# RmSchaffert/ACCV-Lab

Measured on AMD Instinct MI355X. Metric: heatmap frames/sec (1920x1080 fp32, ragged N_obj in [1,128], fused clear+draw), higher is better.
Workload: dtype f32

## Files before the change

accv-lab_amd/csrc/draw_heatmap.hip:

```cpp
#include <hip/hip_runtime.h>
#include <hip/hip_ext.h>

#include <algorithm>
#include <atomic>
#include <climits>
#include <cstdint>
#include <cstring>
#include <type_traits>

#include "accv_common.h"
#include "splat_common.h"
#include "splat_stamps.h"
#include "splat_tile.h"
#include "splat_small.h"
#include "splat_lanes.h"
#include "heatmap_prep.h"

namespace {

void note_dispatch(const char* kernel, int px, int r, bool clear, int sm, const dim3& grid, const dim3& block)
{
    snprintf(accv::dispatch_buffer(), 256, "%s<PX=%d,R=%d,CLEAR=%d,SM=%d> grid(%u,%u,%u) block(%u)", kernel, px, r, clear ? 1 : 0,
             sm, grid.x, grid.y, grid.z, block.x);
}

struct LaunchEvents {
    hipEvent_t start = nullptr, stop = nullptr;
};
LaunchEvents& launch_events()
{
    static thread_local LaunchEvents ev;
    return ev;
}
LaunchEvents take_launch_events()
{
    const LaunchEvents ev = launch_events();
    launch_events() = LaunchEvents{};
    return ev;
}
template <class K>
inline void launch_maybe_timed(K kernel, const dim3& grid, const dim3& block, hipStream_t stream, const LaunchEvents& ev,
                               const SplatParams& p)
{
    if (ev.start || ev.stop)
        hipExtLaunchKernelGGL(kernel, grid, block, 0, stream, ev.start, ev.stop, 0, p);
    else
        hipLaunchKernelGGL(kernel, grid, block, 0, stream, p);
}
template <class F>
void with_variant(bool clear, bool write_through, F&& f)
{
    using Plain = std::integral_constant<int, kStorePlain>;
    using WriteThrough = std::integral_constant<int, kStoreWriteThrough>;
    if (clear && write_through)
        f(std::true_type{}, WriteThrough{});
    else if (clear)
        f(std::true_type{}, Plain{});
    else if (write_through)
        f(std::false_type{}, WriteThrough{});
    else
        f(std::false_type{}, Plain{});
}

int launch_splat_small(SplatParams p, long long planes, bool clear, bool write_through, hipStream_t stream, const LaunchEvents& ev)
{
    p.tiles_x = (p.W + 127) / 128;
    p.tiles_y = (p.H + 15) / 16;
    p.n_tiles = planes * p.tiles_x * p.tiles_y;
    if (p.n_tiles == 0) return ACCV_OK;
    dim3 grid;
    p.grid3d = (planes <= 65535 && p.tiles_y <= 65535) ? 1 : 0;
    if (p.grid3d) {
        grid = dim3((unsigned)p.tiles_x, (unsigned)p.tiles_y, (unsigned)planes);
    } else {
        if (p.n_tiles > INT_MAX) return accv::fail(ACCV_EINVAL, "draw_heatmap: %lld tiles exceed the grid limit", p.n_tiles);
        grid = dim3((unsigned)p.n_tiles);
    }
    with_variant(clear, write_through, [&](auto CL, auto SM) {
        launch_maybe_timed(splat_small_kernel<CL, SM>, grid, dim3(64), stream, ev, p);
    });
    note_dispatch("splat_small_kernel", 4, 8, clear, write_through ? kStoreWriteThrough : kStorePlain, grid, dim3(64));
    return accv::check_launch("draw_heatmap small-splat kernel");
}

template <int PX, int R>
int launch_splat(SplatParams p, long long planes, bool clear, int sm, hipStream_t stream, const LaunchEvents& ev)
{
    p.tiles_x = (p.W + 32 * PX - 1) / (32 * PX);
    p.tiles_y = (p.H + 2 * R - 1) / (2 * R);
    p.n_tiles = planes * p.tiles_x * p.tiles_y;
    if (p.n_tiles == 0) return ACCV_OK;
    const int groups_x = (p.tiles_x + kWavesPerGroup - 1) / kWavesPerGroup;
    dim3 grid, block(kWavesPerGroup * 64);
    p.grid3d = (planes <= 65535 && p.tiles_y <= 65535) ? 1 : 0;
    if (p.grid3d) {
        grid = dim3((unsigned)groups_x, (unsigned)p.tiles_y, (unsigned)planes);
    } else {
        const long long groups = (p.n_tiles + kWavesPerGroup - 1) / kWavesPerGroup;
        if (groups > INT_MAX) return accv::fail(ACCV_EINVAL, "draw_heatmap: %lld tiles exceed the grid limit", p.n_tiles);
        grid = dim3((unsigned)groups);
    }
    attach_splat_stamps(p);
    if (PX == 1 || (sm == kStoreAdaptive && clear)) sm = kStorePlain;
    if (sm == kStoreAdaptive) {
        if constexpr (PX == 4) launch_maybe_timed(splat_kernel<PX, R, false, kStoreAdaptive>, grid, block, stream, ev, p);
    } else {
        with_variant(clear, sm == kStoreWriteThrough, [&](auto CL, auto SM) {
            if constexpr (PX == 4 || SM == kStorePlain) launch_maybe_timed(splat_kernel<PX, R, CL, SM>, grid, block, stream, ev, p);
        });
    }
    note_dispatch("splat_kernel", PX, R, clear, sm, grid, block);
    return accv::check_launch("draw_heatmap splat kernel");
}

long long compute_units()
{
    static std::atomic<int> cached[64];
    int dev = 0;
    if (hipGetDevice(&dev) != hipSuccess || dev < 0 || dev >= 64) return 0;
    int v = cached[dev].load(std::memory_order_relaxed);
    if (v == 0) {
        int n = 0;
        if (hipDeviceGetAttribute(&n, hipDeviceAttributeMultiprocessorCount, dev) != hipSuccess || n <= 0) return 0;
        cached[dev].store(n, std::memory_order_relaxed);
        v = n;
    }
    return v;
}

int dispatch_splat(SplatParams p, long long planes, bool clear, unsigned flags, hipStream_t stream, const LaunchEvents& ev)
{
    const bool small_hint = (flags & ACCV_HM_SMALL_RADII) != 0;
    const bool vec4 = (p.W % 4 == 0) && ((reinterpret_cast<uintptr_t>(p.hm) & 15u) == 0);
    const bool plane_fits_rsrc = (size_t)p.H * p.W * sizeof(float) < ((size_t)1 << 31);
    int nt;
    if (flags & ACCV_HM_WRITE_THROUGH)
        nt = kStoreWriteThrough;
    else if (flags & ACCV_HM_PLAIN_STORES)
        nt = kStorePlain;
    else
        nt = clear ? kStorePlain : kStoreAdaptive;
    if (nt != kStorePlain && !plane_fits_rsrc) nt = kStorePlain;
    p.dense_area = 0.75f * (float)p.H * (float)p.W;
    int rows = (flags & ACCV_HM_TILE_ROWS_16) ? 16 : 8;
    if (!(flags & (ACCV_HM_TILE_ROWS_8 | ACCV_HM_TILE_ROWS_16)) && clear && vec4 && !small_hint) {
        const long long cus = compute_units();
        const long long tx = (p.W + 127) / 128;
        const long long tiles8 = planes * tx * ((p.H + 15) / 16), tiles16 = planes * tx * ((p.H + 31) / 32);
        if (cus > 0 && tiles8 > 24 * cus && tiles16 <= 16 * cus) rows = 16;
    }
    if (!p.labels) p.labels = p.radii;
    if (!vec4) return launch_splat<1, 8>(p, planes, clear, kStorePlain, stream, ev);
    if (small_hint) return launch_splat_small(p, planes, clear, nt == kStoreWriteThrough, stream, ev);
    if (rows == 16) return launch_splat<4, 16>(p, planes, clear, nt, stream, ev);
    return launch_splat<4, 8>(p, planes, clear, nt, stream, ev);
}

int check_common(int h, int w, const char* who)
{
    if (h < 0 || w < 0) return accv::fail(ACCV_EINVAL, "%s: negative heatmap extent %dx%d", who, h, w);
    if (h > (1 << 29) || w > (1 << 29))
        return accv::fail(ACCV_EINVAL, "%s: heatmap extent %dx%d exceeds 2^29 per dimension", who, h, w);
    return ACCV_OK;
}

inline void coarse_scales_first(MultiParams& mp)
{
    std::stable_sort(mp.scale, mp.scale + mp.n_scales,
                     [](const SplatParams& a, const SplatParams& b) { return a.n_tiles < b.n_tiles; });
    long long tiles = 0;
    for (int i = 0; i < mp.n_scales; ++i) {
        mp.tile_begin[i] = tiles;
        tiles += mp.scale[i].n_tiles;
    }
    mp.tile_begin[mp.n_scales] = tiles;
}
inline void seal_tile_prefix(MultiParams& mp)
{
    for (int i = mp.n_scales + 1; i <= kMaxScales; ++i) mp.tile_begin[i] = mp.tile_begin[mp.n_scales];
}

inline int multiscale_store_mode(unsigned flags) { return (flags & ACCV_HM_WRITE_THROUGH) ? kStoreWriteThrough : kStorePlain; }

constexpr const char* kPerScaleNote = " (use the per-scale calls otherwise)";
long long setup_scales(MultiParams& mp, const SplatParams& proto, float* const* heatmaps, const int* heights, const int* widths,
                       const float* strides, int num_scales, int batch, int tile_h, unsigned flags, const char* who,
                       const char* map_note)
{
    long long tiles = 0;
    int used = 0;
    for (int i = 0; i < num_scales; ++i) {
        if (int rc = check_common(heights[i], widths[i], who)) return rc;
        if (!(strides[i] > 0.0f)) return accv::fail(ACCV_EINVAL, "%s: stride %d is not positive", who, i);
        if (heights[i] == 0 || widths[i] == 0) continue;
        if (!heatmaps[i]) return accv::fail(ACCV_EINVAL, "%s: heatmap %d is null", who, i);
        if (widths[i] % 4 != 0 || (reinterpret_cast<uintptr_t>(heatmaps[i]) & 15u) ||
            (size_t)heights[i] * widths[i] * sizeof(float) >= ((size_t)1 << 31))
            return accv::fail(ACCV_EINVAL, "%s: map %d needs a width that is a multiple of 4, a 16-byte aligned base and planes "
                                           "below 2 GiB%s", who, i, map_note);
        SplatParams& p = mp.scale[used];
        p = proto;
        p.hm = heatmaps[i];
        p.H = heights[i];
        p.W = widths[i];
        p.stride = strides[i];
        p.tiles_x = (p.W + 127) / 128;
        p.tiles_y = (p.H + tile_h - 1) / tile_h;
        p.n_tiles = (long long)batch * p.tiles_x * p.tiles_y;
        p.grid3d = 0;
        mp.tile_begin[used] = tiles;
        tiles += p.n_tiles;
        ++used;
    }
    mp.n_scales = used;
    mp.tile_begin[used] = tiles;
    if (!(flags & ACCV_HM_CALLER_SCALE_ORDER)) coarse_scales_first(mp);
    seal_tile_prefix(mp);
    return tiles;
}

int check_scale_arrays(const char* who, float* const* heatmaps, const int* heights, const int* widths, const float* strides,
                       int num_scales)
{
    if (num_scales < 1 || num_scales > kMaxScales)
        return accv::fail(ACCV_EINVAL, "%s: 1..%d scales supported, got %d", who, kMaxScales, num_scales);
    if (!heatmaps || !heights || !widths || !strides) return accv::fail(ACCV_EINVAL, "%s: null array", who);
    return ACCV_OK;
}
int check_scale_counts(const char* who, int batch, int per_sample, const char* what)
{
    if (batch < 0 || per_sample < 0) return accv::fail(ACCV_EINVAL, "%s: negative count", who);
    if (per_sample > (1 << 30)) return accv::fail(ACCV_EINVAL, "%s: more than 2^30 %s per sample", who, what);
    return ACCV_OK;
}
SplatParams multiscale_proto(const void* counts, int n_max, float diameter_to_sigma_factor, float k_scale, unsigned flags)
{
    SplatParams proto{};
    proto.counts = counts;
    proto.n_max = n_max;
    proto.factor = diameter_to_sigma_factor;
    proto.k = k_scale;
    proto.counts_i64 = (flags & ACCV_HM_COUNTS_I64) ? 1 : 0;
    return proto;
}

}

extern "C" {

int accv_draw_heatmap_time_next_launch(void* start_event, void* stop_event)
{
    launch_events() = LaunchEvents{static_cast<hipEvent_t>(start_event), static_cast<hipEvent_t>(stop_event)};
    return ACCV_OK;
}

size_t accv_draw_heatmap_flat_workspace_bytes(int num_planes, int num_objects)
{
    if (num_planes < 0 || num_objects < 0) return 0;
    return accv::align_up((size_t)num_planes * 4, 16) + accv::align_up(((size_t)num_planes + 1) * 4, 16) +
           accv::align_up((size_t)num_objects * 8, 16) + accv::align_up((size_t)num_objects * 4, 16) + 16;
}

int accv_draw_heatmap_flat_f32(float* heatmaps, int num_planes, int height, int width, const int32_t* centers,
                               const int32_t* radii, const int32_t* heatmap_idxes, int num_objects,
                               float diameter_to_sigma_factor, float k_scale, unsigned flags, void* workspace,
                               size_t workspace_bytes, void* stream_)
{
    hipStream_t stream = static_cast<hipStream_t>(stream_);
    const LaunchEvents ev = take_launch_events();
    if (int rc = check_common(height, width, "draw_heatmap")) return rc;
    if (num_planes < 0 || num_objects < 0) return accv::fail(ACCV_EINVAL, "draw_heatmap: negative count");
    if (num_objects > (1 << 30)) return accv::fail(ACCV_EINVAL, "draw_heatmap: more than 2^30 objects");
    const bool clear = (flags & ACCV_HM_CLEAR) != 0;
    if (num_planes == 0 || height == 0 || width == 0) return ACCV_OK;
    if (!heatmaps) return accv::fail(ACCV_EINVAL, "draw_heatmap: heatmap pointer is null");
    if (num_objects > 0 && (!centers || !radii || !heatmap_idxes))
        return accv::fail(ACCV_EINVAL, "draw_heatmap: null object array");
    if (num_objects == 0 && !clear) return ACCV_OK;
    const size_t need = accv_draw_heatmap_flat_workspace_bytes(num_planes, num_objects);
    if (!workspace || workspace_bytes < need || (reinterpret_cast<uintptr_t>(workspace) & 15u))
        return accv::fail(ACCV_EWORKSPACE, "draw_heatmap: workspace needs %zu aligned bytes, got %zu", need,
                          workspace_bytes);

    char* ws = static_cast<char*>(workspace);
    int* cnt = reinterpret_cast<int*>(ws);
    int* off = reinterpret_cast<int*>(ws + accv::align_up((size_t)num_planes * 4, 16));
    char* sc_raw = reinterpret_cast<char*>(off) + accv::align_up(((size_t)num_planes + 1) * 4, 16);
    int2* sorted_centers = reinterpret_cast<int2*>(sc_raw);
    int32_t* sorted_radii = reinterpret_cast<int32_t*>(sc_raw + accv::align_up((size_t)num_objects * 8, 16));

    if (num_planes <= kBinSmallPlanes && num_objects <= kBinSmallObjects) {
        hipLaunchKernelGGL(bin_small_kernel, dim3(1), dim3(1024), 0, stream, heatmap_idxes, num_objects, num_planes,
                           reinterpret_cast<const int2*>(centers), radii, off, sorted_centers, sorted_radii);
    } else {
        if (hipMemsetAsync(cnt, 0, (size_t)num_planes * 4, stream) != hipSuccess)
            return accv::fail(ACCV_ELAUNCH, "draw_heatmap: memset of the bin counters failed");
        const int nb = num_objects > 0 ? min((num_objects + 255) / 256, 1024) : 1;
        if (num_objects > 0)
            hipLaunchKernelGGL(bin_count_kernel, dim3(nb), dim3(256), 0, stream, heatmap_idxes, num_objects, num_planes, cnt);
        hipLaunchKernelGGL(bin_scan_kernel, dim3(1), dim3(1024), 0, stream, cnt, off, num_planes);
        if (num_objects > 0)
            hipLaunchKernelGGL(bin_fill_kernel, dim3(nb), dim3(256), 0, stream, heatmap_idxes, num_objects, num_planes, off,
                               cnt, reinterpret_cast<const int2*>(centers), radii, sorted_centers, sorted_radii);
    }
    if (int rc = accv::check_launch("draw_heatmap binning")) return rc;

    SplatParams p{};
    p.hm = heatmaps;
    p.centers = reinterpret_cast<const int32_t*>(sorted_centers);
    p.radii = sorted_radii;
    p.plane_off = off;
    p.H = height;
    p.W = width;
    p.factor = diameter_to_sigma_factor;
    p.k = k_scale;
    return dispatch_splat(p, num_planes, clear, flags, stream, ev);
}

int accv_draw_heatmap_batched_f32(float* heatmap, int batch, int num_classes, int height, int width,
                                  const int32_t* centers, const int32_t* radii, const void* counts,
                                  const int32_t* labels, int max_num_targets, float diameter_to_sigma_factor,
                                  float k_scale, unsigned flags, void* stream_)
{
    hipStream_t stream = static_cast<hipStream_t>(stream_);
    const LaunchEvents ev = take_launch_events();
    if (int rc = check_common(height, width, "draw_heatmap_batched")) return rc;
    if (batch < 0 || max_num_targets < 0 || num_classes < 0)
        return accv::fail(ACCV_EINVAL, "draw_heatmap_batched: negative count");
    if (max_num_targets > (1 << 30))
        return accv::fail(ACCV_EINVAL, "draw_heatmap_batched: more than 2^30 objects per sample");
    if (batch == 0 || height == 0 || width == 0) return ACCV_OK;
    if (max_num_targets > 0 && (num_classes > 0) != (labels != nullptr))
        return accv::fail(ACCV_EINVAL, "draw_heatmap_batched: labels and num_classes must be given together");
    if (!heatmap) return accv::fail(ACCV_EINVAL, "draw_heatmap_batched: heatmap pointer is null");
    if (!counts) return accv::fail(ACCV_EINVAL, "draw_heatmap_batched: counts pointer is null");
    if (max_num_targets > 0 && (!centers || !radii))
        return accv::fail(ACCV_EINVAL, "draw_heatmap_batched: null object array");
    const bool clear = (flags & ACCV_HM_CLEAR) != 0;
    if (max_num_targets == 0 && !clear) return ACCV_OK;

    SplatParams p{};
    p.hm = heatmap;
    p.centers = centers;
    p.radii = radii;
    p.labels = labels;
    p.counts = counts;
    p.H = height;
    p.W = width;
    p.n_max = max_num_targets;
    p.n_classes = num_classes;
    p.factor = diameter_to_sigma_factor;
    p.k = k_scale;
    p.counts_i64 = (flags & ACCV_HM_COUNTS_I64) ? 1 : 0;
    const long long planes = (long long)batch * (num_classes > 0 ? num_classes : 1);
    return dispatch_splat(p, planes, clear, flags, stream, ev);
}

}

namespace {

struct FusedLaneShape {
    bool ok;
    int p2_shift;
};
FusedLaneShape fused_lane_shape(const int* heights, const int* widths, int num_scales, int batch, int lanes, int points,
                                int num_samples)
{
    FusedLaneShape out{false, 0};
    if (lanes < 1 || points < 1 || points > 64 || num_samples < 1 || num_samples > (1 << 20) || batch < 1) return out;
    int sh = 2;
    while ((1 << sh) < points) ++sh;
    if (((long long)lanes << sh) > kLaneRounds * 64) return out;
    if ((long long)num_samples * 2 > (long long)std::max(points - 1, 1) << sh) return out;
    long long tiles = 0, coarse = 0;
    for (int i = 0; i < num_scales; ++i) {
        if (heights[i] <= 0 || widths[i] <= 0) continue;
        const long long nt = (long long)batch * ((widths[i] + 127) / 128) * ((heights[i] + 15) / 16);
        tiles += nt;
        if ((double)batch * lanes * num_samples >= 24.0 * (double)nt) coarse += nt;
    }
    if (tiles == 0 || 2 * coarse >= tiles) return out;
    out.ok = true;
    out.p2_shift = sh;
    return out;
}

int draw_multiscale_impl(float* const* heatmaps, const int* heights, const int* widths, const float* strides, int num_scales,
                         int batch, const float* centers_xy, const float* boxes_xyxy, const void* counts, int max_num_targets,
                         float diameter_to_sigma_factor, float k_scale, unsigned flags, const WaveSamplerParams* sampler,
                         hipStream_t stream)
{
    (void)take_launch_events();
    auto sampler_only = [&]() -> int {
        if (!sampler) return ACCV_OK;
        TargetsParams tp{};
        tp.sp = *sampler;
        seal_tile_prefix(tp.mp);
        hipLaunchKernelGGL((splat_multi_sampler_kernel<true, kStorePlain>), dim3((unsigned)sampler->n_polylines), dim3(64), 0, stream, tp);
        note_dispatch("splat_multi_sampler_kernel", 4, 8, true, kStorePlain, dim3((unsigned)sampler->n_polylines), dim3(64));
        return accv::check_launch("draw_heatmap multi-scale splat + sampler kernel");
    };
    constexpr const char* who = "draw_heatmap_multiscale";
    if (int rc = check_scale_arrays(who, heatmaps, heights, widths, strides, num_scales)) return rc;
    if (int rc = check_scale_counts(who, batch, max_num_targets, "objects")) return rc;
    if (batch == 0) return sampler_only();
    if (!counts) return accv::fail(ACCV_EINVAL, "draw_heatmap_multiscale: counts pointer is null");
    if (max_num_targets > 0 && (!centers_xy || !boxes_xyxy))
        return accv::fail(ACCV_EINVAL, "draw_heatmap_multiscale: null object array");
    if ((reinterpret_cast<uintptr_t>(boxes_xyxy) & 15u) || (reinterpret_cast<uintptr_t>(centers_xy) & 7u))
        return accv::fail(ACCV_EINVAL, "draw_heatmap_multiscale: centres need 8-byte and boxes 16-byte alignment");
    const bool clear = (flags & ACCV_HM_CLEAR) != 0;
    if (max_num_targets == 0 && !clear) return sampler_only();

    SplatParams proto = multiscale_proto(counts, max_num_targets, diameter_to_sigma_factor, k_scale, flags);
    proto.centers_f = centers_xy;
    proto.boxes_f = boxes_xyxy;
    MultiParams mp{};
    const long long tiles = setup_scales(mp, proto, heatmaps, heights, widths, strides, num_scales, batch, 2 * kBoxTileR,
                                         flags, who, kPerScaleNote);
    if (tiles < 0) return (int)tiles;
    if (tiles == 0) return sampler_only();
    if (tiles + (sampler ? sampler->n_polylines : 0) > INT_MAX)
        return accv::fail(ACCV_EINVAL, "draw_heatmap_multiscale: %lld tiles exceed the grid limit", tiles);
    const int sm = multiscale_store_mode(flags);
    if (sampler) {
        TargetsParams tp{};
        tp.mp = mp;
        tp.sp = *sampler;
        const dim3 grid((unsigned)(tiles + sampler->n_polylines)), block(64);
        with_variant(clear, sm == kStoreWriteThrough, [&](auto CL, auto SM) {
            hipLaunchKernelGGL((splat_multi_sampler_kernel<CL, SM>), grid, block, 0, stream, tp);
        });
        note_dispatch("splat_multi_sampler_kernel", 4, 8, clear, sm, grid, block);
        return accv::check_launch("draw_heatmap multi-scale splat + sampler kernel");
    }
    const dim3 grid((unsigned)tiles), block(64);
    with_variant(clear, sm == kStoreWriteThrough, [&](auto CL, auto SM) {
        hipLaunchKernelGGL((splat_multi_kernel<CL, SM>), grid, block, 0, stream, mp);
    });
    note_dispatch("splat_multi_kernel", 4, 8, clear, sm, grid, block);
    return accv::check_launch("draw_heatmap multi-scale splat kernel");
}

}

extern "C" {

int accv_draw_heatmap_multiscale_f32(float* const* heatmaps, const int* heights, const int* widths, const float* strides,
                                     int num_scales, int batch, const float* centers_xy, const float* boxes_xyxy,
                                     const void* counts, int max_num_targets, float diameter_to_sigma_factor,
                                     float k_scale, unsigned flags, void* stream_)
{
    return draw_multiscale_impl(heatmaps, heights, widths, strides, num_scales, batch, centers_xy, boxes_xyxy, counts,
                                max_num_targets, diameter_to_sigma_factor, k_scale, flags, nullptr, static_cast<hipStream_t>(stream_));
}

int accv_draw_heatmap_multiscale_sample_f32(float* const* heatmaps, const int* heights, const int* widths, const float* strides,
                                            int num_scales, int batch, const float* centers_xy, const float* boxes_xyxy,
                                            const void* counts, int max_num_targets, float diameter_to_sigma_factor,
                                            float k_scale, unsigned flags, const float* polylines_xy, int num_polylines,
                                            int points, const void* point_counts, int num_samples, float* samples,
                                            float* group_boxes, void* stream_)
{
    if (num_polylines < 0) return accv::fail(ACCV_EINVAL, "draw_heatmap_multiscale_sample: negative polyline count");
    if (points < 1 || points > 64)
        return accv::fail(ACCV_EINVAL, "draw_heatmap_multiscale_sample: 1..64 points per polyline (wave-level sampler), got %d",
                          points);
    if (num_samples < 64 || num_samples % 64 != 0 || num_samples > (1 << 20))
        return accv::fail(ACCV_EINVAL, "draw_heatmap_multiscale_sample: the number of samples must be a multiple of 64 up to 2^20 "
                                       "(one group box per 64 samples), got %d", num_samples);
    if (num_polylines > 0 && (!polylines_xy || !samples || !group_boxes))
        return accv::fail(ACCV_EINVAL, "draw_heatmap_multiscale_sample: null polylines / samples / group_boxes");
    if ((reinterpret_cast<uintptr_t>(polylines_xy) & 7u) || (reinterpret_cast<uintptr_t>(samples) & 7u) ||
        (reinterpret_cast<uintptr_t>(group_boxes) & 15u))
        return accv::fail(ACCV_EINVAL, "draw_heatmap_multiscale_sample: polylines / samples need 8-byte, group boxes 16-byte alignment");
    WaveSamplerParams sp{};
    sp.points = reinterpret_cast<const float2*>(polylines_xy);
    sp.point_counts = point_counts;
    sp.samples = reinterpret_cast<float2*>(samples);
    sp.boxes = reinterpret_cast<float4*>(group_boxes);
    sp.n_polylines = num_polylines;
    sp.P = points;
    sp.S = num_samples;
    sp.counts_i64 = (flags & ACCV_HM_POINT_COUNTS_I64) ? 1 : 0;
    return draw_multiscale_impl(heatmaps, heights, widths, strides, num_scales, batch, centers_xy, boxes_xyxy, counts,
                                max_num_targets, diameter_to_sigma_factor, k_scale, flags, num_polylines > 0 ? &sp : nullptr,
                                static_cast<hipStream_t>(stream_));
}

size_t accv_draw_points_workspace_bytes(int batch, int num_points)
{
    if (batch < 0 || num_points < 0) return 0;
    return (size_t)batch * (size_t)((num_points + 63) / 64) * sizeof(float4) + 16;
}

int accv_draw_points_multiscale_f32(float* const* heatmaps, const int* heights, const int* widths, const float* strides,
                                    int num_scales, int batch, const float* points_xy, const void* counts, int num_points,
                                    int radius, float diameter_to_sigma_factor, float k_scale, unsigned flags,
                                    void* workspace, size_t workspace_bytes, void* stream_)
{
    hipStream_t stream = static_cast<hipStream_t>(stream_);
    (void)take_launch_events();
    constexpr const char* who = "draw_points_multiscale";
    if (int rc = check_scale_arrays(who, heatmaps, heights, widths, strides, num_scales)) return rc;
    if (int rc = check_scale_counts(who, batch, num_points, "points")) return rc;
    if (batch == 0) return ACCV_OK;
    if (!counts) return accv::fail(ACCV_EINVAL, "draw_points_multiscale: counts pointer is null");
    if (num_points > 0 && !points_xy) return accv::fail(ACCV_EINVAL, "draw_points_multiscale: null point array");
    if (reinterpret_cast<uintptr_t>(points_xy) & 7u)
        return accv::fail(ACCV_EINVAL, "draw_points_multiscale: points need 8-byte alignment");
    const bool clear = (flags & ACCV_HM_CLEAR) != 0;
    if (num_points == 0 && !clear) return ACCV_OK;
    const size_t need = accv_draw_points_workspace_bytes(batch, num_points);
    if (!workspace || workspace_bytes < need || (reinterpret_cast<uintptr_t>(workspace) & 15u))
        return accv::fail(ACCV_EWORKSPACE, "draw_points_multiscale: workspace needs %zu aligned bytes, got %zu", need,
                          workspace_bytes);
    const int n_groups = (num_points + 63) / 64;

    SplatParams proto = multiscale_proto(counts, num_points, diameter_to_sigma_factor, k_scale, flags);
    proto.centers_f = points_xy;
    proto.boxes_f = static_cast<const float*>(workspace);
    proto.radius = radius;
    proto.n_groups = n_groups;
    MultiParams mp{};
    const long long tiles = setup_scales(mp, proto, heatmaps, heights, widths, strides, num_scales, batch, kSmallTH,
                                         flags, who, kPerScaleNote);
    if (tiles <= 0) return (int)tiles;
    if (tiles > INT_MAX) return accv::fail(ACCV_EINVAL, "draw_points_multiscale: %lld tiles exceed the grid limit", tiles);
    const long long total_groups = (long long)batch * n_groups;
    if (total_groups > INT_MAX) return accv::fail(ACCV_EINVAL, "draw_points_multiscale: too many point groups");
    if (total_groups > 0 && !(flags & ACCV_HM_GROUP_BOXES_GIVEN))
        hipLaunchKernelGGL(group_boxes_kernel, dim3((unsigned)total_groups), dim3(64), 0, stream,
                           reinterpret_cast<const float2*>(points_xy), num_points, n_groups, total_groups,
                           static_cast<float4*>(workspace));
    long long coarse_tiles = 0;
    for (int i = 0; i < mp.n_scales; ++i)
        if ((double)batch * num_points >= 24.0 * (double)mp.scale[i].n_tiles) coarse_tiles += mp.scale[i].n_tiles;
    const bool heavy = 2 * coarse_tiles >= tiles;
    const int sm = multiscale_store_mode(flags);
    const dim3 grid((unsigned)tiles), block(heavy ? 256 : 64);
    with_variant(clear, sm == kStoreWriteThrough, [&](auto CL, auto SM) {
        if (heavy)
            hipLaunchKernelGGL((splat_points_multi_kernel<CL, SM, 4>), grid, block, 0, stream, mp);
        else
            hipLaunchKernelGGL((splat_points_multi_kernel<CL, SM, 1>), grid, block, 0, stream, mp);
    });
    note_dispatch("splat_points_multi_kernel", 4, 8, clear, sm, grid, block);
    return accv::check_launch("draw_heatmap multi-scale point splat kernel");
}

int accv_draw_polylines_fused_applicable(const int* heights, const int* widths, int num_scales, int batch, int lanes,
                                         int points, int num_samples)
{
    if (!heights || !widths || num_scales < 1 || num_scales > kMaxScales) return 0;
    return fused_lane_shape(heights, widths, num_scales, batch, lanes, points, num_samples).ok ? 1 : 0;
}

int accv_draw_polylines_multiscale_f32(float* const* heatmaps, const int* heights, const int* widths, const float* strides,
                                       int num_scales, int batch, const float* polylines_xy, int lanes, int points,
                                       const void* point_counts, const void* lane_counts, int num_samples, int radius,
                                       float diameter_to_sigma_factor, float k_scale, unsigned flags, void* stream_)
{
    hipStream_t stream = static_cast<hipStream_t>(stream_);
    constexpr const char* who = "draw_polylines_multiscale";
    if (int rc = check_scale_arrays(who, heatmaps, heights, widths, strides, num_scales)) return rc;
    if (batch < 0) return accv::fail(ACCV_EINVAL, "draw_polylines_multiscale: negative batch");
    if (batch == 0) return ACCV_OK;
    if (radius < 0) return accv::fail(ACCV_EINVAL, "draw_polylines_multiscale: negative radius");
    const FusedLaneShape shape = fused_lane_shape(heights, widths, num_scales, batch, lanes, points, num_samples);
    if (!shape.ok)
        return accv::fail(ACCV_EINVAL, "draw_polylines_multiscale: shape outside the fused kernel (1..64 points per polyline, "
                                       "lanes x points rounded up to a power of two <= %d, samples <= (points - 1) x that power "
                                       "of two / 2, fine scales in the majority: accv_draw_polylines_fused_applicable); use "
                                       "accv_polyline_sample_boxes + accv_draw_points_multiscale_f32", kLaneRounds * 64);
    if (!polylines_xy || !lane_counts)
        return accv::fail(ACCV_EINVAL, "draw_polylines_multiscale: null polylines / lane_counts");
    if (reinterpret_cast<uintptr_t>(polylines_xy) & 7u)
        return accv::fail(ACCV_EINVAL, "draw_polylines_multiscale: polylines need 8-byte alignment");
    const bool clear = (flags & ACCV_HM_CLEAR) != 0;

    SplatParams proto = multiscale_proto(lane_counts, lanes, diameter_to_sigma_factor, k_scale, flags);
    proto.radius = radius;
    FusedLaneParams fp{};
    const long long tiles = setup_scales(fp.mp, proto, heatmaps, heights, widths, strides, num_scales, batch, kSmallTH,
                                         flags, who, "");
    if (tiles <= 0) return (int)tiles;
    if (tiles > INT_MAX) return accv::fail(ACCV_EINVAL, "draw_polylines_multiscale: %lld tiles exceed the grid limit", tiles);
    fp.lp.points = reinterpret_cast<const float2*>(polylines_xy);
    fp.lp.point_counts = point_counts;
    fp.lp.L = lanes;
    fp.lp.P = points;
    fp.lp.S = num_samples;
    fp.lp.p2_shift = shape.p2_shift;
    fp.lp.counts_i64 = (flags & ACCV_HM_POINT_COUNTS_I64) ? 1 : 0;
    const int sm = multiscale_store_mode(flags);
    const dim3 grid((unsigned)tiles), block(64);
    with_variant(clear, sm == kStoreWriteThrough, [&](auto CL, auto SM) {
        hipLaunchKernelGGL((lane_raster_multi_kernel<CL, SM>), grid, block, 0, stream, fp);
    });
    note_dispatch("lane_raster_multi_kernel", 4, 8, clear, sm, grid, block);
    return accv::check_launch("draw_heatmap fused lane raster kernel");
}

int accv_heatmap_targets_from_boxes_f32(const float* centers_xy, const float* boxes_xyxy, long long num_objects,
                                        float stride, int32_t* out_centers, int32_t* out_radii, void* stream_)
{
    hipStream_t stream = static_cast<hipStream_t>(stream_);
    if (num_objects < 0) return accv::fail(ACCV_EINVAL, "targets_from_boxes: negative count");
    if (num_objects == 0) return ACCV_OK;
    if (!centers_xy || !boxes_xyxy || !out_centers || !out_radii)
        return accv::fail(ACCV_EINVAL, "targets_from_boxes: null pointer");
    if ((reinterpret_cast<uintptr_t>(boxes_xyxy) & 15u) || (reinterpret_cast<uintptr_t>(centers_xy) & 7u) ||
        (reinterpret_cast<uintptr_t>(out_centers) & 7u))
        return accv::fail(ACCV_EINVAL, "targets_from_boxes: centres need 8-byte and boxes 16-byte alignment");
    const unsigned grid = (unsigned)std::min<long long>((num_objects + 255) / 256, 4096);
    hipLaunchKernelGGL(targets_from_boxes_kernel, dim3(grid), dim3(256), 0, stream,
                       reinterpret_cast<const float2*>(centers_xy), reinterpret_cast<const float4*>(boxes_xyxy),
                       num_objects, stride, reinterpret_cast<int2*>(out_centers), out_radii);
    return accv::check_launch("targets_from_boxes");
}

int accv_heatmap_targets_from_points_f32(const float* points_xy, long long num_points, float stride, int radius,
                                         int32_t* out_centers, int32_t* out_radii, void* stream_)
{
    hipStream_t stream = static_cast<hipStream_t>(stream_);
    if (num_points < 0) return accv::fail(ACCV_EINVAL, "targets_from_points: negative count");
    if (num_points == 0) return ACCV_OK;
    if (!points_xy || !out_centers || !out_radii) return accv::fail(ACCV_EINVAL, "targets_from_points: null pointer");
    if ((reinterpret_cast<uintptr_t>(points_xy) & 7u) || (reinterpret_cast<uintptr_t>(out_centers) & 7u))
        return accv::fail(ACCV_EINVAL, "targets_from_points: points and centres need 8-byte alignment");
    const unsigned grid = (unsigned)std::min<long long>((num_points + 255) / 256, 4096);
    hipLaunchKernelGGL(targets_from_points_kernel, dim3(grid), dim3(256), 0, stream,
                       reinterpret_cast<const float2*>(points_xy), num_points, stride, radius,
                       reinterpret_cast<int2*>(out_centers), out_radii);
    return accv::check_launch("targets_from_points");
}

int accv_fill_f32(float* dst, size_t count, float value, void* stream_)
{
    hipStream_t stream = static_cast<hipStream_t>(stream_);
    if (count == 0) return ACCV_OK;
    if (!dst) return accv::fail(ACCV_EINVAL, "fill: null pointer");
    size_t head = 0;
    while (((reinterpret_cast<uintptr_t>(dst + head)) & 15u) && head < count) ++head;
    if (head) hipLaunchKernelGGL(fill_tail_kernel, dim3(1), dim3(64), 0, stream, dst, head, value);
    const size_t n4 = (count - head) / 4;
    for (size_t done = 0; done < n4;) {
        const size_t part = std::min(n4 - done, (size_t)0x7fffffff * 256);
        hipLaunchKernelGGL(fill_kernel, dim3((unsigned)((part + 255) / 256)), dim3(256), 0, stream,
                           reinterpret_cast<float4*>(dst + head) + done, part, value);
        done += part;
    }
    const size_t tail = count - head - n4 * 4;
    if (tail) hipLaunchKernelGGL(fill_tail_kernel, dim3(1), dim3(64), 0, stream, dst + head + n4 * 4, tail, value);
    return accv::check_launch("fill");
}

}
```

accv-lab_amd/csrc/splat_common.h:

```cpp
#pragma once
#include <hip/hip_runtime.h>

#include <cstdint>

#include "accv_common.h"

namespace {

constexpr int kWavesPerGroup = 1;
constexpr int kBoxTileR = 8;
constexpr int kCand = 64;
constexpr float kLog2e = 1.4426950408889634f;

constexpr int kSrcObjects = 0;
constexpr int kSrcFloatBoxes = 1;
constexpr int kSrcPoints = 2;
constexpr int kStorePlain = 0;
constexpr int kStoreWriteThrough = 4;
constexpr int kStoreAdaptive = 5;

struct SplatParams {
    float* hm;
    const int32_t* centers;
    const int32_t* radii;
    const int32_t* labels;
    const void* counts;
    const int32_t* plane_off;
    int H, W;
    int n_max;
    int n_classes;
    int tiles_x, tiles_y;
    long long n_tiles;
    float factor, k;
    int counts_i64;
    int grid3d;
    float dense_area;
    const float* centers_f;
    const float* boxes_f;
    float stride;
    int radius, n_groups;
#ifdef ACCV_SPLAT_STAMPS
    unsigned long long* stamps;
    long long stamp_records;
#endif
};

constexpr int kMaxScales = 4;
struct MultiParams {
    SplatParams scale[kMaxScales];
    long long tile_begin[kMaxScales + 1];
    int n_scales;
};

struct __attribute__((aligned(16))) Hit {
    int x, y;
    float c2;
    unsigned box;
};

template <int PX>
struct Vec;
typedef float vfloat4 __attribute__((ext_vector_type(4)));
template <>
struct Vec<4> {
    using type = vfloat4;
};
template <>
struct Vec<1> {
    using type = float;
};

__device__ __forceinline__ float raw_exp2(float x) { return __builtin_amdgcn_exp2f(x); }

__device__ __forceinline__ float max_skip_nan(float acc, float v)
{
    float r;
    asm("v_max_f32 %0, %1, %2" : "=v"(r) : "v"(acc), "v"(v));
    return r;
}

struct TileCtx {
    int tx0, ty0, tx1, ty1;
    long long plane;
    const int2* centers2;
    const int32_t* radii;
    const int32_t* labels;
    const float2* centers_f;
    const float4* boxes_f;
    float4 box0;
    float stride;
    int radius;
    int n, cls;
};

template <bool SCALAR_COUNT = false>
__device__ __forceinline__ void plane_objects(const SplatParams& p, TileCtx& t);

template <int TW, int TH, int WPG, bool SCALAR_COUNT = false>
__device__ __forceinline__ bool locate_tile(const SplatParams& p, int wave, TileCtx& t, long long linear_group)
{
    int tx, ty;
    if (p.grid3d) {
        tx = blockIdx.x * WPG + wave;
        ty = blockIdx.y;
        t.plane = blockIdx.z;
        if (tx >= p.tiles_x) return false;
    } else {
        const long long tile = linear_group * WPG + wave;
        if (tile >= p.n_tiles) return false;
        if (p.n_tiles <= 0x7fffffffll) {
            const unsigned t32 = (unsigned)tile, t2 = t32 / (unsigned)p.tiles_x;
            tx = (int)(t32 - t2 * (unsigned)p.tiles_x);
            const unsigned pl = t2 / (unsigned)p.tiles_y;
            ty = (int)(t2 - pl * (unsigned)p.tiles_y);
            t.plane = pl;
        } else {
            tx = (int)(tile % p.tiles_x);
            const long long t2 = tile / p.tiles_x;
            ty = (int)(t2 % p.tiles_y);
            t.plane = t2 / p.tiles_y;
        }
    }
    t.tx0 = tx * TW;
    t.ty0 = ty * TH;
    t.tx1 = min(t.tx0 + TW, p.W);
    t.ty1 = min(t.ty0 + TH, p.H);
    plane_objects<SCALAR_COUNT>(p, t);
    return true;
}

template <bool SCALAR_COUNT>
__device__ __forceinline__ void plane_objects(const SplatParams& p, TileCtx& t)
{
    long long obj_base;
    t.cls = -1;
    if (p.plane_off) {
        const int o0 = p.plane_off[t.plane];
        obj_base = o0;
        t.n = p.plane_off[t.plane + 1] - o0;
    } else {
        long long s = t.plane;
        if (p.n_classes > 0) {
            s = t.plane / p.n_classes;
            t.cls = (int)(t.plane - s * p.n_classes);
        }
        long long cnt;
        if constexpr (SCALAR_COUNT) {
            if (p.n_groups > 0)
                t.box0 = reinterpret_cast<const float4*>(p.boxes_f)[t.plane * p.n_groups + min((int)(threadIdx.x & 63), p.n_groups - 1)];
            using ConstI32 = const __attribute__((address_space(4))) int;
            using ConstI64 = const __attribute__((address_space(4))) long long;
            const uintptr_t base = reinterpret_cast<uintptr_t>(p.counts);
            cnt = p.counts_i64 ? reinterpret_cast<ConstI64*>(base)[s] : (long long)reinterpret_cast<ConstI32*>(base)[s];
        } else {
            cnt = p.counts_i64 ? ((const long long*)p.counts)[s] : (long long)((const int*)p.counts)[s];
        }
        t.n = (int)max(0ll, min(cnt, (long long)p.n_max));
        obj_base = s * p.n_max;
    }
    t.centers2 = reinterpret_cast<const int2*>(p.centers) + obj_base;
    t.radii = p.radii + obj_base;
    t.labels = p.labels + obj_base;
    t.centers_f = reinterpret_cast<const float2*>(p.centers_f) + obj_base;
    t.boxes_f = reinterpret_cast<const float4*>(p.boxes_f) + (p.n_groups > 0 ? (t.plane * p.n_groups) : obj_base);
    t.stride = p.stride;
    t.radius = p.radius;
}

struct Cand {
    int x, y, r, label;
};
template <int SRC = kSrcObjects>
__device__ __forceinline__ Cand cull_load(const TileCtx& t, int base, int lane)
{
    const int cc = min(base + lane, t.n - 1);
    if constexpr (SRC == kSrcFloatBoxes) {
        const float2 c = t.centers_f[cc];
        const float4 b = t.boxes_f[cc];
        const float m = fminf(fminf(c.x - b.x, c.y - b.y), fminf(b.z - c.x, b.w - c.y));
        const bool pow2 = (__float_as_uint(t.stride) & 0x007fffffu) == 0u && t.stride > 1.0e-30f && t.stride < 1.0e30f;
        if (pow2) {
            const float inv = 1.0f / t.stride;
            int r = (int)ceilf(m * inv);
            if (r < 1) r = 1;
            return Cand{(int)(c.x * inv), (int)(c.y * inv), r, 0};
        }
        int r = (int)ceilf(__fdiv_rn(m, t.stride));
        if (r < 1) r = 1;
        return Cand{(int)__fdiv_rn(c.x, t.stride), (int)__fdiv_rn(c.y, t.stride), r, 0};
    } else if constexpr (SRC == kSrcPoints) {
        const float2 c = t.centers_f[cc];
        const bool bad = (c.x != c.x) || (c.y != c.y);
        if (bad) return Cand{0, 0, -1, 0};
        return Cand{(int)__fdiv_rn(c.x, t.stride), (int)__fdiv_rn(c.y, t.stride), t.radius, 0};
    } else {
        const int2 cxy = t.centers2[cc];
        return Cand{cxy.x, cxy.y, t.radii[cc], t.labels[cc]};
    }
}
__device__ __forceinline__ unsigned long long cull_test(const TileCtx& t, int base, int lane, const Cand& c)
{
    constexpr int kClampXY = 1 << 29, kClampR = 1 << 30;
    const int xc = min(max(c.x, -kClampXY), kClampXY), yc = min(max(c.y, -kClampXY), kClampXY);
    const int rc = min(c.r, kClampR);
    const bool hit = (base + lane < t.n) && (t.cls < 0 || c.label == t.cls) && c.r >= 0 && xc - rc < t.tx1 &&
                     xc + rc >= t.tx0 && yc - rc < t.ty1 && yc + rc >= t.ty0;
    return __ballot(hit);
}
template <int SRC = kSrcObjects>
__device__ __forceinline__ unsigned long long cull_round(const TileCtx& t, int base, int lane, int& x, int& y, int& r)
{
    const Cand c = cull_load<SRC>(t, base, lane);
    x = c.x;
    y = c.y;
    r = c.r;
    return cull_test(t, base, lane, c);
}

__device__ __forceinline__ float hit_exponent_scale(const SplatParams& p, int r)
{
    const float sigma = (float)(2 * r + 1) / p.factor;
    return kLog2e / (2.0f * sigma * sigma);
}
__device__ __forceinline__ Hit make_hit(const SplatParams& p, const TileCtx& t, int x, int y, int r, float c2);
__device__ __forceinline__ Hit make_hit(const SplatParams& p, const TileCtx& t, int x, int y, int r)
{
    return make_hit(p, t, x, y, r, hit_exponent_scale(p, r));
}
__device__ __forceinline__ Hit make_hit(const SplatParams& p, const TileCtx& t, int x, int y, int r, float c2)
{
    const long long x0 = (long long)x - min(x, r), x1 = (long long)x + min((long long)p.W - x, (long long)r + 1);
    const long long y0 = (long long)y - min(y, r), y1 = (long long)y + min((long long)p.H - y, (long long)r + 1);
    const long long xlo = max(x0, (long long)t.tx0) - t.tx0, xhi = min(x1, (long long)t.tx1) - t.tx0;
    const long long ylo = max(y0, (long long)t.ty0) - t.ty0, yhi = min(y1, (long long)t.ty1) - t.ty0;
    unsigned box = 0;
    if (xhi > xlo && yhi > ylo) box = (unsigned)xlo | ((unsigned)xhi << 8) | ((unsigned)ylo << 16) | ((unsigned)yhi << 24);
    return Hit{x, y, c2, box};
}

__device__ __forceinline__ float max3_skip_nan(float acc, float a, float b)
{
    float r;
    asm("v_max3_f32 %0, %1, %2, %3" : "=v"(r) : "v"(acc), "v"(a), "v"(b));
    return r;
}

__device__ __forceinline__ int scale_of_group(const MultiParams& mp, long long group, long long& first)
{
    int s = 0;
    first = 0;
#pragma unroll
    for (int i = 1; i < kMaxScales; ++i) {
        const long long begin = mp.tile_begin[i];
        if (group >= begin) {
            s = i;
            first = begin;
        }
    }
    return s;
}
template <typename T>
__device__ __forceinline__ void pin_scalar(T& v)
{
    asm volatile("" : "+s"(v));
}
__device__ __forceinline__ SplatParams preload_params(const SplatParams& src)
{
    SplatParams p = src;
    asm volatile("" ::"s"(p.hm), "s"(p.counts), "s"(p.centers_f), "s"(p.boxes_f));
    pin_scalar(p.H);
    pin_scalar(p.W);
    pin_scalar(p.n_max);
    pin_scalar(p.n_classes);
    pin_scalar(p.tiles_x);
    pin_scalar(p.tiles_y);
    pin_scalar(p.n_tiles);
    pin_scalar(p.factor);
    pin_scalar(p.k);
    pin_scalar(p.counts_i64);
    pin_scalar(p.grid3d);
    pin_scalar(p.dense_area);
    pin_scalar(p.stride);
    pin_scalar(p.radius);
    pin_scalar(p.n_groups);
    return p;
}

constexpr int kDppQuad0 = 0x00, kDppQuad1 = 0x55, kDppQuad2 = 0xAA, kDppQuad3 = 0xFF;
constexpr int kDppRowShr = 0x110;
constexpr int kDppWaveShl1 = 0x130, kDppWaveShr1 = 0x138;
template <int CTRL>
__device__ __forceinline__ float dpp_f(float old, float src)
{
    return __int_as_float(__builtin_amdgcn_update_dpp(__float_as_int(old), __float_as_int(src), CTRL, 0xf, 0xf, false));
}
template <int CTRL>
__device__ __forceinline__ int dpp_i(int old, int src)
{
    return __builtin_amdgcn_update_dpp(old, src, CTRL, 0xf, 0xf, false);
}

}
```

accv-lab_amd/csrc/splat_stamps.h:

```cpp
#pragma once

namespace {

template <bool ON>
struct PhaseStamps {
    __device__ __forceinline__ void start() {}
    __device__ __forceinline__ void cull() {}
    __device__ __forceinline__ void table() {}
    __device__ __forceinline__ void accumulate() {}
    __device__ __forceinline__ void record(const SplatParams&, long long, int, int, int) {}
};

#ifdef ACCV_SPLAT_STAMPS
constexpr bool kSplatStampsBuilt = true;
__device__ __forceinline__ unsigned long long phase_stamp()
{
    __builtin_amdgcn_sched_barrier(0);
    const unsigned long long v = __builtin_amdgcn_s_memrealtime();
    __builtin_amdgcn_sched_barrier(0);
    return v;
}
__device__ __forceinline__ unsigned xcc_id()
{
    unsigned v;
    asm volatile("s_getreg_b32 %0, hwreg(HW_REG_XCC_ID, 0, 4)" : "=s"(v));
    return v;
}

template <>
struct PhaseStamps<true> {
    unsigned long long st_start = 0, st_prev = 0, st_cull = 0, st_table = 0, st_acc = 0;
    int rounds = 0;

    __device__ __forceinline__ unsigned long long lap()
    {
        const unsigned long long now = phase_stamp(), d = now - st_prev;
        st_prev = now;
        return d;
    }
    __device__ __forceinline__ void start() { st_start = st_prev = phase_stamp(); }
    __device__ __forceinline__ void cull()
    {
        st_cull += lap();
        ++rounds;
    }
    __device__ __forceinline__ void table() { st_table += lap(); }
    __device__ __forceinline__ void accumulate() { st_acc += lap(); }
    __device__ __forceinline__ void record(const SplatParams& p, long long rec, int lane, int n, int total_hits)
    {
        const unsigned long long done = phase_stamp();
        if (lane == 0 && p.stamps && rec < p.stamp_records) {
            unsigned long long* o = p.stamps + 8 * rec;
            o[0] = st_start;
            o[1] = st_cull;
            o[2] = st_table;
            o[3] = st_acc;
            o[4] = st_prev;
            o[5] = (unsigned long long)n;
            o[6] = done;
            o[7] = (unsigned long long)(unsigned)total_hits | ((unsigned long long)rounds << 16) | ((unsigned long long)xcc_id() << 32);
        }
    }
};

unsigned long long* g_splat_stamps = nullptr;
long long g_splat_stamp_records = 0;
inline void attach_splat_stamps(SplatParams& p)
{
    p.stamps = g_splat_stamps;
    p.stamp_records = g_splat_stamp_records;
}
#else
constexpr bool kSplatStampsBuilt = false;
inline void attach_splat_stamps(SplatParams&) {}
#endif

}

#ifdef ACCV_SPLAT_STAMPS
extern "C" void accv_debug_splat_stamps(void* buffer, long long records)
{
    g_splat_stamps = static_cast<unsigned long long*>(buffer);
    g_splat_stamp_records = buffer ? records : 0;
}
#endif
```

accv-lab_amd/csrc/splat_tile.h:

```cpp
#pragma once

namespace {

template <int PX, int R, bool CLEAR, int SM, int WPG, int SRC>
__device__ __forceinline__ void splat_body(const SplatParams& p, long long linear_group)
{
    constexpr int kWavesPerGroup = WPG;
    constexpr int TW = 32 * PX;
    constexpr int TH = 2 * R;
    static_assert(R % 4 == 0, "row registers are fetched four at a time");

    __shared__ Hit s_hit[kWavesPerGroup][kCand];
    __shared__ __attribute__((aligned(16))) float s_ey[kWavesPerGroup][kCand][TH];

    constexpr bool kSharedColumns = CLEAR && SRC == kSrcObjects && PX == 4;
    PhaseStamps<kSplatStampsBuilt && CLEAR && SRC == kSrcObjects && PX == 4> stamps;
    stamps.start();
    const int lane = threadIdx.x & 63;
    const int wave = __builtin_amdgcn_readfirstlane(threadIdx.x >> 6);
    TileCtx t;
    if (!locate_tile<TW, TH, kWavesPerGroup>(p, wave, t, linear_group)) return;
    const int tx0 = t.tx0, ty0 = t.ty0, n = t.n;
    const long long plane = t.plane;

    const int sub = lane >> 5;
    const int col0 = tx0 + (lane & 31) * PX;

    float acc[R][PX];
    const float init = CLEAR ? 0.0f : __builtin_nanf("");
#pragma unroll
    for (int i = 0; i < R; ++i)
#pragma unroll
        for (int c = 0; c < PX; ++c) acc[i][c] = init;

    int total_hits = 0;
    float cover = 0.0f;

    for (int base = 0; base < n; base += kCand) {
        int x, y, r;
        const unsigned long long m = cull_round<SRC>(t, base, lane, x, y, r);
        if constexpr (SM == kStoreAdaptive) {
            const float dia = (float)(2 * min(max(r, 0), 1 << 20) + 1);
            cover += (base + lane < n) ? dia * dia : 0.0f;
        }
        const bool hit = (m >> lane) & 1ull;
        const int nh = __popcll(m);
        stamps.cull();
        if (nh == 0) continue;
        if constexpr (!CLEAR) {
            if (total_hits == 0 && col0 < p.W) {
                const float* plane_rd = p.hm + (size_t)plane * (size_t)p.H * (size_t)p.W;
#pragma unroll
                for (int i = 0; i < R; ++i) {
                    const int row = ty0 + sub * R + i;
                    if (row < p.H) {
                        if constexpr (PX == 4) {
                            const vfloat4 o = *reinterpret_cast<const vfloat4*>(plane_rd + (size_t)row * p.W + col0);
                            acc[i][0] = o.x;
                            acc[i][1] = o.y;
                            acc[i][2] = o.z;
                            acc[i][3] = o.w;
                        } else {
                            acc[i][0] = plane_rd[(size_t)row * p.W + col0];
                        }
                    }
                }
            }
        }
        if (hit) s_hit[wave][__popcll(m & ((1ull << lane) - 1ull))] = make_hit(p, t, x, y, r);
        __builtin_amdgcn_fence(__ATOMIC_RELEASE, "wavefront");
        __builtin_amdgcn_fence(__ATOMIC_ACQUIRE, "wavefront");

        for (int t = lane; t < nh * TH; t += 64) {
            const int h = t / TH, rr = t % TH;
            const Hit hy = s_hit[wave][h];
            const float d = (float)(ty0 + rr - hy.y);
            const float v = p.k * raw_exp2(-(d * d) * hy.c2);
            const unsigned ylo = (hy.box >> 16) & 255u, yhi = hy.box >> 24;
            s_ey[wave][h][rr] = ((unsigned)rr >= ylo && (unsigned)rr < yhi) ? v : __builtin_nanf("");
        }
        __builtin_amdgcn_fence(__ATOMIC_RELEASE, "wavefront");
        __builtin_amdgcn_fence(__ATOMIC_ACQUIRE, "wavefront");
        stamps.table();

        const unsigned colr0 = (unsigned)(lane & 31) * PX;
        auto column_factors = [&](const Hit& hx, float (&ex)[PX]) {
            const unsigned xlo = hx.box & 255u, xhi = (hx.box >> 8) & 255u;
#pragma unroll
            for (int c = 0; c < PX; ++c) {
                const float d = (float)(col0 + c - hx.x);
                const float e = raw_exp2(-(d * d) * hx.c2);
                ex[c] = (colr0 + c >= xlo && colr0 + c < xhi) ? e : __builtin_nanf("");
            }
        };
        [[maybe_unused]] auto column_factors_shared = [&](const Hit& hx, float (&ex)[PX]) {
            if constexpr (PX == 4) {
                const unsigned xlo = hx.box & 255u, xhi = (hx.box >> 8) & 255u;
                unsigned f[2];
#pragma unroll
                for (int j = 0; j < 2; ++j) {
                    const int c = 2 * sub + j;
                    const float d = (float)(col0 + c - hx.x);
                    const float e = raw_exp2(-(d * d) * hx.c2);
                    f[j] = __float_as_uint((colr0 + c >= xlo && colr0 + c < xhi) ? e : __builtin_nanf(""));
                }
#pragma unroll
                for (int j = 0; j < 2; ++j) {
                    const auto sw = __builtin_amdgcn_permlane32_swap(f[j], f[j], false, false);
                    ex[j] = __uint_as_float(sw[0]);
                    ex[2 + j] = __uint_as_float(sw[1]);
                }
            }
        };
        int h = 0;
        for (; CLEAR && h + 1 < nh; h += 2) {
            float exa[PX], exb[PX];
            if constexpr (kSharedColumns) {
                column_factors_shared(s_hit[wave][h], exa);
                column_factors_shared(s_hit[wave][h + 1], exb);
            } else {
                column_factors(s_hit[wave][h], exa);
                column_factors(s_hit[wave][h + 1], exb);
            }
#pragma unroll
            for (int q = 0; q < R / 4; ++q) {
                const float4 a4 = *reinterpret_cast<const float4*>(&s_ey[wave][h][sub * R + 4 * q]);
                const float4 b4 = *reinterpret_cast<const float4*>(&s_ey[wave][h + 1][sub * R + 4 * q]);
                const float eya[4] = {a4.x, a4.y, a4.z, a4.w}, eyb[4] = {b4.x, b4.y, b4.z, b4.w};
#pragma unroll
                for (int i = 0; i < 4; ++i)
#pragma unroll
                    for (int c = 0; c < PX; ++c)
                        acc[4 * q + i][c] = max3_skip_nan(acc[4 * q + i][c], exa[c] * eya[i], exb[c] * eyb[i]);
            }
        }
        for (; h < nh; ++h) {
            float ex[PX];
            if constexpr (kSharedColumns)
                column_factors_shared(s_hit[wave][h], ex);
            else
                column_factors(s_hit[wave][h], ex);
#pragma unroll
            for (int q = 0; q < R / 4; ++q) {
                const float4 e4 = *reinterpret_cast<const float4*>(&s_ey[wave][h][sub * R + 4 * q]);
                const float ey[4] = {e4.x, e4.y, e4.z, e4.w};
#pragma unroll
                for (int i = 0; i < 4; ++i)
#pragma unroll
                    for (int c = 0; c < PX; ++c) acc[4 * q + i][c] = max_skip_nan(acc[4 * q + i][c], ex[c] * ey[i]);
            }
        }
        total_hits += nh;
        stamps.accumulate();
        __builtin_amdgcn_fence(__ATOMIC_RELEASE, "wavefront");
        __builtin_amdgcn_fence(__ATOMIC_ACQUIRE, "wavefront");
    }

    if (!CLEAR && total_hits == 0) return;
    if (col0 >= p.W) return;

    using V = typename Vec<PX>::type;
    float* plane_ptr = p.hm + (size_t)plane * (size_t)p.H * (size_t)p.W;
    bool write_through = SM == kStoreWriteThrough;
    if constexpr (SM == kStoreAdaptive && PX == 4) {
#pragma unroll
        for (int d = 32; d >= 1; d >>= 1) cover += __shfl_xor(cover, d);
        write_through = cover >= p.dense_area;
    }
#pragma unroll
    for (int i = 0; i < R; ++i) {
        const int row = ty0 + sub * R + i;
        if (row >= p.H) break;
        V* dst = reinterpret_cast<V*>(plane_ptr + (size_t)row * p.W + col0);
        V out;
        if constexpr (PX == 4)
            out = V{acc[i][0], acc[i][1], acc[i][2], acc[i][3]};
        else
            out = acc[i][0];
        if constexpr (SM != kStorePlain && PX == 4) {
            if (write_through) {
                const auto rsrc = __builtin_amdgcn_make_buffer_rsrc(plane_ptr, 0, (int)((size_t)p.H * p.W * 4), 0x00020000);
                __builtin_amdgcn_raw_buffer_store_b128(out, rsrc, (int)(((size_t)row * p.W + col0) * 4), 0, 18);
            } else {
                *dst = out;
            }
        } else {
            *dst = out;
        }
    }
    stamps.record(p, (plane * p.tiles_y + ty0 / TH) * p.tiles_x + tx0 / TW, lane, n, total_hits);
}

template <int PX, int R, bool CLEAR, int SM, int WPG = kWavesPerGroup>
__global__ __launch_bounds__(WPG * 64) void splat_kernel(const SplatParams p)
{
    splat_body<PX, R, CLEAR, SM, WPG, kSrcObjects>(p, blockIdx.x);
}

template <bool CLEAR, int SM>
__global__ __launch_bounds__(64) void splat_multi_kernel(const MultiParams mp)
{
    long long first;
    const int s = scale_of_group(mp, blockIdx.x, first);
    splat_body<4, kBoxTileR, CLEAR, SM, 1, kSrcFloatBoxes>(mp.scale[s], (long long)blockIdx.x - first);
}

}
```

Before: 713,200.

## Add one-round splat kernel with prefetched first candidate and staggered row mapping

Adds a specialized clear+draw kernel for the 16-row tile path. It loads the first candidate object per lane early, inside plane_objects, so that load overlaps the tile setup. It also hoists the parameter pointers into scalar registers and remaps tile rows across planes with a staggered offset, likely to spread work or memory traffic across XCDs or channels. The stamps debug record gains a hardware ID field. The new path adds template variants and code size, and it only applies when no plane offsets are given and n_max is positive.

```diff
diff --git a/accv-lab_amd/csrc/draw_heatmap.hip b/accv-lab_amd/csrc/draw_heatmap.hip
--- a/accv-lab_amd/csrc/draw_heatmap.hip
+++ b/accv-lab_amd/csrc/draw_heatmap.hip
@@ -83,8 +83,12 @@
     return accv::check_launch("draw_heatmap small-splat kernel");
 }
 
+void launch_one_round(bool write_through, const dim3& grid, const dim3& block, hipStream_t stream, const LaunchEvents& ev,
+                      const SplatParams& p);
+
 template <int PX, int R>
-int launch_splat(SplatParams p, long long planes, bool clear, int sm, hipStream_t stream, const LaunchEvents& ev)
+int launch_splat(SplatParams p, long long planes, bool clear, int sm, hipStream_t stream, const LaunchEvents& ev,
+                 bool one_round = false)
 {
     p.tiles_x = (p.W + 32 * PX - 1) / (32 * PX);
     p.tiles_y = (p.H + 2 * R - 1) / (2 * R);
@@ -106,6 +110,9 @@
         if constexpr (PX == 4) launch_maybe_timed(splat_kernel<PX, R, false, kStoreAdaptive>, grid, block, stream, ev, p);
     } else {
         with_variant(clear, sm == kStoreWriteThrough, [&](auto CL, auto SM) {
+            if constexpr (PX == 4 && R == 16 && CL) {
+                if (one_round) return launch_one_round(SM == kStoreWriteThrough, grid, block, stream, ev, p);
+            }
             if constexpr (PX == 4 || SM == kStorePlain) launch_maybe_timed(splat_kernel<PX, R, CL, SM>, grid, block, stream, ev, p);
         });
     }
@@ -143,16 +150,20 @@
     if (nt != kStorePlain && !plane_fits_rsrc) nt = kStorePlain;
     p.dense_area = 0.75f * (float)p.H * (float)p.W;
     int rows = (flags & ACCV_HM_TILE_ROWS_16) ? 16 : 8;
+    bool one_round = false;
     if (!(flags & (ACCV_HM_TILE_ROWS_8 | ACCV_HM_TILE_ROWS_16)) && clear && vec4 && !small_hint) {
         const long long cus = compute_units();
         const long long tx = (p.W + 127) / 128;
         const long long tiles8 = planes * tx * ((p.H + 15) / 16), tiles16 = planes * tx * ((p.H + 31) / 32);
-        if (cus > 0 && tiles8 > 24 * cus && tiles16 <= 16 * cus) rows = 16;
+        if (cus > 0 && tiles8 > 24 * cus && tiles16 <= 16 * cus) {
+            rows = 16;
+            one_round = !p.plane_off && p.n_max > 0;
+        }
     }
     if (!p.labels) p.labels = p.radii;
     if (!vec4) return launch_splat<1, 8>(p, planes, clear, kStorePlain, stream, ev);
     if (small_hint) return launch_splat_small(p, planes, clear, nt == kStoreWriteThrough, stream, ev);
-    if (rows == 16) return launch_splat<4, 16>(p, planes, clear, nt, stream, ev);
+    if (rows == 16) return launch_splat<4, 16>(p, planes, clear, nt, stream, ev, one_round);
     return launch_splat<4, 8>(p, planes, clear, nt, stream, ev);
 }
 
@@ -658,3 +669,16 @@
 }
 
 }
+
+namespace {
+
+void launch_one_round(bool write_through, const dim3& grid, const dim3& block, hipStream_t stream, const LaunchEvents& ev,
+                      const SplatParams& p)
+{
+    if (write_through)
+        launch_maybe_timed(splat_one_round_kernel<kStoreWriteThrough>, grid, block, stream, ev, p);
+    else
+        launch_maybe_timed(splat_one_round_kernel<kStorePlain>, grid, block, stream, ev, p);
+}
+
+}
diff --git a/accv-lab_amd/csrc/splat_common.h b/accv-lab_amd/csrc/splat_common.h
--- a/accv-lab_amd/csrc/splat_common.h
+++ b/accv-lab_amd/csrc/splat_common.h
@@ -4,6 +4,7 @@
 #include <cstdint>
 
 #include "accv_common.h"
+#include "splat_deal.h"
 
 namespace {
 
@@ -79,6 +80,9 @@
     return r;
 }
 
+struct Cand {
+    int x, y, r, label;
+};
 struct TileCtx {
     int tx0, ty0, tx1, ty1;
     long long plane;
@@ -88,15 +92,16 @@
     const float2* centers_f;
     const float4* boxes_f;
     float4 box0;
+    Cand first;
     float stride;
     int radius;
     int n, cls;
 };
 
-template <bool SCALAR_COUNT = false>
+template <bool SCALAR_COUNT = false, bool ONE_ROUND = false>
 __device__ __forceinline__ void plane_objects(const SplatParams& p, TileCtx& t);
 
-template <int TW, int TH, int WPG, bool SCALAR_COUNT = false>
+template <int TW, int TH, int WPG, bool SCALAR_COUNT = false, bool ONE_ROUND = false>
 __device__ __forceinline__ bool locate_tile(const SplatParams& p, int wave, TileCtx& t, long long linear_group)
 {
     int tx, ty;
@@ -104,6 +109,7 @@
         tx = blockIdx.x * WPG + wave;
         ty = blockIdx.y;
         t.plane = blockIdx.z;
+        if constexpr (ONE_ROUND) ty = accv_deal::one_round_row(ty, blockIdx.z, p.tiles_y);
         if (tx >= p.tiles_x) return false;
     } else {
         const long long tile = linear_group * WPG + wave;
@@ -125,16 +131,16 @@
     t.ty0 = ty * TH;
     t.tx1 = min(t.tx0 + TW, p.W);
     t.ty1 = min(t.ty0 + TH, p.H);
-    plane_objects<SCALAR_COUNT>(p, t);
+    plane_objects<SCALAR_COUNT, ONE_ROUND>(p, t);
     return true;
 }
 
-template <bool SCALAR_COUNT>
+template <bool SCALAR_COUNT, bool ONE_ROUND>
 __device__ __forceinline__ void plane_objects(const SplatParams& p, TileCtx& t)
 {
     long long obj_base;
     t.cls = -1;
-    if (p.plane_off) {
+    if (!ONE_ROUND && p.plane_off) {
         const int o0 = p.plane_off[t.plane];
         obj_base = o0;
         t.n = p.plane_off[t.plane + 1] - o0;
@@ -143,6 +149,11 @@
         if (p.n_classes > 0) {
             s = t.plane / p.n_classes;
             t.cls = (int)(t.plane - s * p.n_classes);
+        }
+        if constexpr (ONE_ROUND) {
+            const long long at = s * p.n_max + min((int)(threadIdx.x & 63), p.n_max - 1);
+            const int2 cxy = reinterpret_cast<const int2*>(p.centers)[at];
+            t.first = Cand{cxy.x, cxy.y, p.radii[at], p.labels[at]};
         }
         long long cnt;
         if constexpr (SCALAR_COUNT) {
@@ -167,9 +178,6 @@
     t.radius = p.radius;
 }
 
-struct Cand {
-    int x, y, r, label;
-};
 template <int SRC = kSrcObjects>
 __device__ __forceinline__ Cand cull_load(const TileCtx& t, int base, int lane)
 {
diff --git a/accv-lab_amd/csrc/splat_deal.h b/accv-lab_amd/csrc/splat_deal.h
--- /dev/null
+++ b/accv-lab_amd/csrc/splat_deal.h
@@ -0,0 +1,17 @@
+#pragma once
+
+#if defined(__HIPCC__)
+#define ACCV_DEAL_HD __host__ __device__
+#else
+#define ACCV_DEAL_HD
+#endif
+
+namespace accv_deal {
+
+ACCV_DEAL_HD inline int one_round_row(int y, int z, int tiles_y)
+{
+    const int row = y + ((z >> 1) & 3) * (tiles_y >> 2);
+    return row >= tiles_y ? row - tiles_y : row;
+}
+
+}
diff --git a/accv-lab_amd/csrc/splat_stamps.h b/accv-lab_amd/csrc/splat_stamps.h
--- a/accv-lab_amd/csrc/splat_stamps.h
+++ b/accv-lab_amd/csrc/splat_stamps.h
@@ -24,6 +24,13 @@
 {
     unsigned v;
     asm volatile("s_getreg_b32 %0, hwreg(HW_REG_XCC_ID, 0, 4)" : "=s"(v));
+    return v;
+}
+
+__device__ __forceinline__ unsigned hw_id()
+{
+    unsigned v;
+    asm volatile("s_getreg_b32 %0, hwreg(HW_REG_HW_ID, 0, 16)" : "=s"(v));
     return v;
 }
 
@@ -58,7 +65,8 @@
             o[4] = st_prev;
             o[5] = (unsigned long long)n;
             o[6] = done;
-            o[7] = (unsigned long long)(unsigned)total_hits | ((unsigned long long)rounds << 16) | ((unsigned long long)xcc_id() << 32);
+            o[7] = (unsigned long long)(unsigned)total_hits | ((unsigned long long)rounds << 16) | ((unsigned long long)xcc_id() << 32) |
+                   ((unsigned long long)hw_id() << 36);
         }
     }
 };
diff --git a/accv-lab_amd/csrc/splat_tile.h b/accv-lab_amd/csrc/splat_tile.h
--- a/accv-lab_amd/csrc/splat_tile.h
+++ b/accv-lab_amd/csrc/splat_tile.h
@@ -2,7 +2,7 @@
 
 namespace {
 
-template <int PX, int R, bool CLEAR, int SM, int WPG, int SRC>
+template <int PX, int R, bool CLEAR, int SM, int WPG, int SRC, bool ONE_ROUND = false>
 __device__ __forceinline__ void splat_body(const SplatParams& p, long long linear_group)
 {
     constexpr int kWavesPerGroup = WPG;
@@ -16,10 +16,13 @@
     constexpr bool kSharedColumns = CLEAR && SRC == kSrcObjects && PX == 4;
     PhaseStamps<kSplatStampsBuilt && CLEAR && SRC == kSrcObjects && PX == 4> stamps;
     stamps.start();
+    if constexpr (ONE_ROUND)
+        asm volatile("" ::"s"(p.centers), "s"(p.radii), "s"(p.labels), "s"(p.counts), "s"(p.n_max), "s"(p.n_classes),
+                     "s"(p.counts_i64), "s"(p.grid3d), "s"(p.tiles_x));
     const int lane = threadIdx.x & 63;
     const int wave = __builtin_amdgcn_readfirstlane(threadIdx.x >> 6);
     TileCtx t;
-    if (!locate_tile<TW, TH, kWavesPerGroup>(p, wave, t, linear_group)) return;
+    if (!locate_tile<TW, TH, kWavesPerGroup, false, ONE_ROUND>(p, wave, t, linear_group)) return;
     const int tx0 = t.tx0, ty0 = t.ty0, n = t.n;
     const long long plane = t.plane;
 
@@ -38,7 +41,15 @@
 
     for (int base = 0; base < n; base += kCand) {
         int x, y, r;
-        const unsigned long long m = cull_round<SRC>(t, base, lane, x, y, r);
+        unsigned long long m;
+        if (ONE_ROUND && base == 0) {
+            x = t.first.x;
+            y = t.first.y;
+            r = t.first.r;
+            m = cull_test(t, 0, lane, t.first);
+        } else {
+            m = cull_round<SRC>(t, base, lane, x, y, r);
+        }
         if constexpr (SM == kStoreAdaptive) {
             const float dia = (float)(2 * min(max(r, 0), 1 << 20) + 1);
             cover += (base + lane < n) ? dia * dia : 0.0f;
@@ -188,13 +199,20 @@
             *dst = out;
         }
     }
-    stamps.record(p, (plane * p.tiles_y + ty0 / TH) * p.tiles_x + tx0 / TW, lane, n, total_hits);
+    stamps.record(p, ((p.grid3d ? blockIdx.z : plane) * p.tiles_y + (p.grid3d ? (long long)blockIdx.y : ty0 / TH)) * p.tiles_x + tx0 / TW,
+                  lane, n, total_hits);
 }
 
 template <int PX, int R, bool CLEAR, int SM, int WPG = kWavesPerGroup>
 __global__ __launch_bounds__(WPG * 64) void splat_kernel(const SplatParams p)
 {
     splat_body<PX, R, CLEAR, SM, WPG, kSrcObjects>(p, blockIdx.x);
+}
+
+template <int SM>
+__global__ __launch_bounds__(kWavesPerGroup * 64) void splat_one_round_kernel(const SplatParams p)
+{
+    splat_body<4, 16, true, SM, kWavesPerGroup, kSrcObjects, true>(p, blockIdx.x);
 }
 
 template <bool CLEAR, int SM>
```

After: 713,500, median of 3. Within noise of the previous version (+0.0%).
